# unirestore/UniRestore

Measured on AMD Instinct MI355X. Metric: restored 512x512 images/sec @ 20 denoise steps (whole job), higher is better.
Workload: dtype bf16; 1 GPU; PIR 512x512 batch=8/GPU, 20 DDIM steps, bf16, hipGraph replay (BASELINE.json configs[1]; configs[2] shape for N=8); global_batch=8, per_gpu_batch=8, image=512, denoise_steps=20, parallelism=image-parallel dp1, weights=seeded random init (no checkpoints reachable)

## Files before the change

### include/unirestore_hip.h

```cpp
#ifndef UNIRESTORE_HIP_H
#define UNIRESTORE_HIP_H

#include <stddef.h>
#include <stdint.h>

#ifdef __cplusplus
extern "C" {
#endif

typedef void* ur_stream_t;

enum { UR_OK = 0, UR_E_INVALID = -1, UR_E_UNSUPPORTED = -2, UR_E_LAUNCH = -3, UR_E_WORKSPACE = -4 };

enum { UR_DT_BF16 = 0, UR_DT_F16 = 1 };

enum {
  UR_ACT_NONE = 0,
  UR_ACT_SILU = 1,
  UR_ACT_GELU = 2,
  UR_ACT_GEGLU = 3,
  UR_ACT_GATE = 4,
  UR_ACT_TANH = 5,
  UR_ACT_RELU = 6
};
// ... 16 lines not shown
  const float* ln_stats;
  const float* ln_colsum;
  float ln_eps;
  int ln_dim;
  int ln_parts;
  float* workspace;
  size_t workspace_bytes;
  int N, H, W;
  int C1, ldx, C2, ldx2;
  int Cout, ldw, ldy, ldr;
  int KH, KW, stride, pad_t, pad_l;
  int OH, OW;
  int upsample2x;
  int act;
  int out_f32;
  int n_split, t_rows, t_ld;
  float out_scale;
  int nbatch;
  long long bs_x, bs_x2, bs_w, bs_bias, bs_y, bs_r;
  int k_chunk_major;
  long long bias_img_stride;
  int dtype;
  const void* w_frag;
} ur_conv_desc;

int ur_conv2d_nhwc(const ur_conv_desc* d, ur_stream_t stream);

typedef struct ur_conv_plan {
  int row_stat_parts;
  int gn_parts;
  int gn_fused;
  int prologue_ok;
} ur_conv_plan;
int ur_conv2d_plan(const ur_conv_desc* d, ur_conv_plan* plan);

typedef struct ur_conv_launch_info {
  int launcher;
  int splitk;
  int nk_per_split;
  int reduce;
  int reduce_ri;
  int gn_pass;
  int group_loop;
} ur_conv_launch_info;
int ur_conv2d_plan_launch(const ur_conv_desc* d, ur_conv_launch_info* info);
int ur_conv_launcher_count(void);
const char* ur_conv_launcher_name(int i);

int ur_gemm_bias_act(const void* x, const void* w, const float* bias, const void* residual, void* y, long long M, int N, int K,
                     int ldx, int ldw, int ldy, int ldr, int act, float* workspace, size_t workspace_bytes, int dtype,
                     ur_stream_t stream);
int ur_groupconv3x3_nhwc(const void* x, const void* w, const float* bias, void* y, int N, int H, int W, int Cg, int Cog,
                         int groups, int act, float* workspace, size_t workspace_bytes, int dtype, ur_stream_t stream);

int ur_groupnorm_stats_parts(int N, int HW, int C);
// ... 89 lines not shown
```

### unirestore_amd/build.py

```python
import json
import os
import re
import subprocess
import sys
from concurrent.futures import ThreadPoolExecutor

HERE = os.path.dirname(os.path.abspath(__file__))
CSRC = os.path.join(HERE, "csrc")
LIB = os.environ.get("UR_LIB_OUT") or os.path.join(HERE, "libunirestore_hip.so")
EXTRA = os.environ.get("UR_EXTRA_FLAGS", "").split()
IGEMM_UNITS = ["igemm_v2.hip", "igemm_halo.hip", "igemm_v1a.hip", "igemm_v1b.hip", "igemm_g1.hip"]
SOURCES = [(u, [f"-DUR_TU_F16={t}"], u.replace(".hip", "_f16.o" if t else "_bf16.o")) for u in IGEMM_UNITS for t in (0, 1)] + \
          [("conv_wstream.hip", [f"-DUR_TU_F16={t}"], "conv_wstream_f16.o" if t else "conv_wstream_bf16.o") for t in (0, 1)] + \
          [("attention.hip", [f"-DUR_TU_F16={t}"], "attention_f16.o" if t else "attention_bf16.o") for t in (0, 1)] + \
          [("attention_pp.hip", [f"-DUR_TU_F16={t}"], "attention_pp_f16.o" if t else "attention_pp_bf16.o") for t in (0, 1)] + \
          [("attention512.hip", [f"-DUR_TU_F16={t}"], "attention512_f16.o" if t else "attention512_bf16.o") for t in (0, 1)] + \
          [(u, [], u.replace(".hip", ".o")) for u in ("tchain.hip", "igemm.hip", "norms.hip", "elementwise.hip", "runtime.hip", "metrics.hip")]
FLAGS = ["--offload-arch=gfx950", "-O3", "-std=c++17", "-fPIC", "-Wno-unused-value",
         "-Wno-unused-result"]


def _hipcc():
    for c in ("/opt/rocm/bin/hipcc", "hipcc"):
        if os.path.isabs(c) and os.path.exists(c):
            return c
    return "hipcc"


def needs_build():
    if not os.path.exists(LIB):
        return True
    t = os.path.getmtime(LIB)
    deps = [os.path.join(CSRC, f) for f in os.listdir(CSRC)] + [os.path.join(HERE, "..", "include", "unirestore_hip.h")]
    return any(os.path.getmtime(d) > t for d in deps)
# ... 57 lines not shown
```

### unirestore_amd/capi.py

```python
import ctypes as C
import os

import torch

_HERE = os.path.dirname(os.path.abspath(__file__))
LIB_PATH = os.environ.get("UR_LIB") or os.path.join(_HERE, "libunirestore_hip.so")

UR_ACT_NONE, UR_ACT_SILU, UR_ACT_GELU, UR_ACT_GEGLU, UR_ACT_GATE, UR_ACT_TANH, UR_ACT_RELU = range(7)
UR_DT_BF16, UR_DT_F16 = 0, 1
UR_E_INVALID, UR_E_UNSUPPORTED = -1, -2


class ConvDesc(C.Structure):
    _fields_ = [
        ("x", C.c_void_p), ("x2", C.c_void_p), ("w", C.c_void_p), ("bias", C.c_void_p), ("residual", C.c_void_p),
        ("y", C.c_void_p), ("yt", C.c_void_p), ("gn_part", C.c_void_p), ("gn_ab", C.c_void_p), ("gn_silu", C.c_int),
        ("row_stats", C.c_void_p), ("ln_stats", C.c_void_p), ("ln_colsum", C.c_void_p), ("ln_eps", C.c_float), ("ln_dim", C.c_int), ("ln_parts", C.c_int),
        ("workspace", C.c_void_p),
        ("workspace_bytes", C.c_size_t),
        ("N", C.c_int), ("H", C.c_int), ("W", C.c_int),
        ("C1", C.c_int), ("ldx", C.c_int), ("C2", C.c_int), ("ldx2", C.c_int),
        ("Cout", C.c_int), ("ldw", C.c_int), ("ldy", C.c_int), ("ldr", C.c_int),
        ("KH", C.c_int), ("KW", C.c_int), ("stride", C.c_int), ("pad_t", C.c_int), ("pad_l", C.c_int),
        ("OH", C.c_int), ("OW", C.c_int),
        ("upsample2x", C.c_int), ("act", C.c_int), ("out_f32", C.c_int),
        ("n_split", C.c_int), ("t_rows", C.c_int), ("t_ld", C.c_int),
        ("out_scale", C.c_float),
        ("nbatch", C.c_int),
        ("bs_x", C.c_longlong), ("bs_x2", C.c_longlong), ("bs_w", C.c_longlong), ("bs_bias", C.c_longlong),
        ("bs_y", C.c_longlong), ("bs_r", C.c_longlong), ("k_chunk_major", C.c_int), ("bias_img_stride", C.c_longlong),
        ("dtype", C.c_int), ("w_frag", C.c_void_p),
    ]


class ConvPlan(C.Structure):
    _fields_ = [("row_stat_parts", C.c_int), ("gn_parts", C.c_int), ("gn_fused", C.c_int), ("prologue_ok", C.c_int)]


class ConvLaunchInfo(C.Structure):
    _fields_ = [("launcher", C.c_int), ("splitk", C.c_int), ("nk_per_split", C.c_int), ("reduce", C.c_int), ("reduce_ri", C.c_int),
                ("gn_pass", C.c_int), ("group_loop", C.c_int)]


_P, _I, _F, _LL, _SZ = C.c_void_p, C.c_int, C.c_float, C.c_longlong, C.c_size_t

SIGNATURES = {
    "ur_version": (_I, []),
    "ur_last_error": (C.c_char_p, []),
    "ur_conv2d_nhwc": (_I, [C.POINTER(ConvDesc), _P]),
    "ur_conv2d_plan": (_I, [C.POINTER(ConvDesc), C.POINTER(ConvPlan)]),
    "ur_conv2d_plan_launch": (_I, [C.POINTER(ConvDesc), C.POINTER(ConvLaunchInfo)]),
    "ur_conv_launcher_count": (_I, []),
    "ur_conv_launcher_name": (C.c_char_p, [_I]),
    "ur_gemm_bias_act": (_I, [_P, _P, _P, _P, _P, _LL, _I, _I, _I, _I, _I, _I, _I, _P, _SZ, _I, _P]),
    "ur_groupconv3x3_nhwc": (_I, [_P, _P, _P, _P, _I, _I, _I, _I, _I, _I, _I, _P, _SZ, _I, _P]),
    "ur_groupnorm_stats_parts": (_I, [_I, _I, _I]),
    "ur_groupnorm_ws_bytes": (_SZ, [_I, _I, _I]),
    "ur_groupnorm_ab_bytes": (_SZ, [_I, _I]),
    "ur_groupnorm_stats": (_I, [_P, _P, _I, _I, _I, _I, _P]),
# ... 82 lines not shown
```

### unirestore_amd/csrc/igemm.hip

```cpp
#include "igemm_impl.h"

namespace urk {
#define UR_DECLARE(name)                                                                                             \
  ConvLaunch name##_bf16(void* k, size_t ws_bytes);                                                                 \
  ConvLaunch name##_f16(void* k, size_t ws_bytes);                                                                  \
  static ConvLaunch name(ConvK& k, size_t ws_bytes) { return (k.f16 ? name##_f16 : name##_bf16)(&k, ws_bytes); }
UR_CONV_LAUNCHERS(UR_DECLARE)
#undef UR_DECLARE
}

namespace {

ConvLaunch dispatch_conv(ConvK& k, bool pair, size_t ws_bytes) {
  if (k.KH == 3 && k.stride == 1 && k.pad_t == 1 && k.pad_l == 1 && k.kcm && k.staged_ok_ && !pair && k.nbatch == 1 &&
      k.OW % 32 == 0 && k.OH % 8 == 0 && k.OH == (k.ups ? 2 * k.H : k.H) && k.OW == (k.ups ? 2 * k.W : k.W) && !k.yt) {
    const bool ok128 = k.Cout % 128 == 0, ok160 = k.Cout % 160 == 0;
    const long long tm8 = (long long)k.N * (k.OH / 8) * (k.OW / 32);
    auto eff = [](long long t) { return t <= 128 ? (double)(t * (256 / t)) / 256.0 : (double)t / (double)(((t + 255) / 256) * 256); };
    const bool use160 = ok160 && (!ok128 || eff(tm8 * (k.Cout / 160)) >= eff(tm8 * (k.Cout / 128)));
    const long long tiles8 = tm8 * (use160 ? k.Cout / 160 : k.Cout / 128);
    if ((ok128 || ok160) && tiles8 >= 64) {
      if (use160) return urk::halo_8x32_160(k, ws_bytes);
      return urk::halo_8x32_128(k, ws_bytes);
    }
  }
  if (k.KH == 3 && k.stride == 1 && k.pad_t == 1 && k.pad_l == 1 && k.kcm && !pair && k.nbatch == 1 && !k.ups && k.C2 == 0 &&
      k.Cout <= 32 && k.OW % 32 == 0 && k.OH % 8 == 0 && k.OH == k.H && k.OW == k.W && !k.yt && !k.gn_part && !k.gn_ab && !k.row_stats && !k.ln_stats &&
      !k.bias_img && (long long)k.N * (k.OH / 8) * (k.OW / 32) >= 128)
    return urk::halo_thin_32(k, ws_bytes);
  const bool himg_ups = k.ups && k.OH == 16 && k.OW == 16 && k.H == 8 && k.W == 8;
  if (k.KH == 3 && k.stride == 1 && k.pad_t == 1 && k.pad_l == 1 && k.kcm && k.staged_ok_ && !pair && k.nbatch == 1 &&
// ... 34 lines not shown
    if (k.Cout <= 32) return urk::v1_256x32(k, ws_bytes);
    if (k.Cout <= 64) return urk::v1_128x64(k, ws_bytes);
    if (k.Cout % 160 == 0 && k.Cout % 128 != 0) return g1 && nosplit(128, 160) ? urk::g1_128x160(k, ws_bytes) : urk::v1_128x160(k, ws_bytes);
    return g1 && nosplit(128, 128) ? urk::g1_128x128(k, ws_bytes) : urk::v1_128x128(k, ws_bytes);
  }
  if (k.Cout <= 32) return urk::v2_256x32(k, ws_bytes);
  if (k.Cout <= 64 && !pair) return urk::v2_128x64(k, ws_bytes);
  const bool n160 = !pair && k.Cout % 160 == 0 && k.Cout % 128 != 0;
  const long long big_tiles = (long long)((k.M + 255) / 256) * ((k.Cout + (n160 ? 159 : 127)) / (n160 ? 160 : 128)) * k.nbatch;
  if (g1 && !pair && big_tiles < 256) {
    const long long t160 = k.Cout % 160 == 0 ? (long long)((k.M + 127) / 128) * (k.Cout / 160) : 0;
    const long long t128 = (long long)((k.M + 127) / 128) * ((k.Cout + 127) / 128);
    auto fill = [](long long t) { return t <= 0 ? 0.0 : (double)t / (double)(((t + 255) / 256) * 256); };
    if (t160 >= 200 && fill(t160) >= fill(t128)) return urk::g1_128x160(k, ws_bytes);
    if (t128 >= 200) return urk::g1_128x128(k, ws_bytes);
  }
  if (big_tiles >= 160) {
    if (n160 && g1) return urk::g1_128x160(k, ws_bytes);
    if (n160) return urk::v2_256x160(k, ws_bytes);
    return urk::v2_256x128(k, ws_bytes);
  }
  if (k.Cout % 160 == 0 && k.Cout % 128 != 0 && !pair) return urk::v1_128x160(k, ws_bytes);
  return urk::v1_128x128(k, ws_bytes);
}

}

static int conv_impl(const ur_conv_desc* d, ur_stream_t stream, ur_conv_plan* plan, ur_conv_launch_info* info = nullptr) {
  UR_REQUIRE(d && d->x && d->w, "null x/w");
  UR_REQUIRE(d->KH == d->KW && (d->KH == 1 || d->KH == 3), "only 1x1 and 3x3 kernels");
  UR_REQUIRE(d->C1 > 0 && d->C1 % 8 == 0 && d->C2 % 8 == 0 && d->ldx % 8 == 0, "Cin/ldx must be multiples of 8");
  UR_REQUIRE(d->C2 == 0 || (d->x2 && d->ldx2 % 8 == 0), "virtual concat needs x2");
  UR_REQUIRE(d->Cout > 0 && d->Cout % 4 == 0 && d->ldw % 8 == 0, "Cout%4, ldw%8");
  UR_REQUIRE(d->nbatch >= 1 && d->stride >= 1 && d->OH > 0 && d->OW > 0, "bad dims");
  UR_REQUIRE(d->y || d->yt || d->gn_part, "no output requested");
  UR_REQUIRE_DT(d->dtype);
  const bool pair = d->act == UR_ACT_GEGLU || d->act == UR_ACT_GATE;
  if (pair && d->Cout % 64 != 0)
    return ur::fail(UR_E_UNSUPPORTED, "ur_conv2d_nhwc: pair activations (GEGLU / SimpleGate) need Cout % 64 == 0 (32-row a|g interleave)");
  UR_REQUIRE(!d->y || (d->out_f32 ? d->ldy % 4 == 0 : d->ldy % 4 == 0), "ldy%4");
  UR_REQUIRE(!d->residual || d->ldr % 4 == 0, "ldr%4");
  UR_REQUIRE(!d->yt || (d->t_rows > 0 && d->n_split % 4 == 0 && !pair), "bad transposed-output spec");

  ConvK k;
  k.x = (const uint16_t*)d->x; k.x2 = (const uint16_t*)d->x2; k.w = (const uint16_t*)d->w; k.bias = d->bias;
  k.res = (const uint16_t*)d->residual; k.y = d->y; k.yt = (uint16_t*)d->yt;
// ... 12 lines not shown

  k.kcm = d->k_chunk_major; k.wf = (const uint16_t*)d->w_frag; k.wmajor = 0; k.xgm = 0; k.xbn = 0; k.patch_tw = 0;
  UR_REQUIRE(!k.kcm || (k.Cin % 64 == 0 && d->C1 % 64 == 0), "k_chunk_major needs C1 and C1+C2 to be multiples of 64");
  k.gn_part = d->gn_part; k.gn_ab = d->gn_ab; k.gn_silu = d->gn_silu; k.f16 = d->dtype == UR_DT_F16; k.gn_fused = 0; k.gn_parts = 0;
  k.ln_parts = d->ln_parts;
  k.row_stats = d->row_stats; k.ln_stats = d->ln_stats; k.ln_colsum = d->ln_colsum; k.ln_eps = d->ln_eps; k.ln_dim = d->ln_dim;
  UR_REQUIRE(!d->ln_stats || (d->ln_colsum && d->ln_dim > 0), "ln_stats needs ln_colsum / ln_dim");
  UR_REQUIRE(!(d->bias_img_stride && (pair || d->ln_stats || d->yt)), "per-image bias rows do not combine with pair activations / LayerNorm folding / transposed columns");
  k.staged_ok_ = (d->y ? (!d->out_f32 && ((d->ldy | d->bs_y) & 7) == 0) : d->gn_part != nullptr) &&
                 (!d->residual || ((d->ldr | d->bs_r) & 7) == 0);
  UR_REQUIRE(!d->gn_part || (!d->out_f32 && !d->yt), "gn_part needs a plain 16-bit output (or none)");
  hipStream_t s = (hipStream_t)stream;
  const double flops = 2.0 * k.M * (double)k.Cout * k.Ktot * k.nbatch;
  const double bytes = 2.0 * ((double)k.M * k.Cin + (double)k.Cout * k.Ktot + (double)k.M * k.Cout) * k.nbatch;
  const char* fam = d->KH == 3 ? "conv3x3_igemm" : "gemm1x1_igemm";
  static const bool prof_shapes = getenv("UR_PROF_SHAPES") != nullptr;
  if (prof_shapes) {
    static std::map<std::string, int> interned;
    char buf[128];
    snprintf(buf, sizeof buf, "%s M%d N%d K%d s%d u%d b%d a%d", d->KH == 3 ? "c3" : "g1", k.M, k.Cout, k.Ktot, d->stride, d->upsample2x,
             k.nbatch, d->act);
    fam = interned.emplace(buf, 0).first->first.c_str();
  }
  const ConvLaunch launch = dispatch_conv(k, pair, d->workspace_bytes);
  const bool group_loop = k.nbatch > 1 && d->KH == 3 && k.kcm && k.stride == 1 && !pair && !k.gn_part && !k.row_stats && !k.ln_stats &&
                          !k.yt && !k.gn_ab && !k.out_f32 && k.staged_ok_ && k.Cout % 128 == 0 && !k.bias_img && k.C2 == 0;
  auto group_k = [&](int b) {
    ConvK kb = k;
    kb.nbatch = 1;
    kb.x = k.x + b * k.bs_x; kb.w = k.w + b * k.bs_w; kb.bias = k.bias ? k.bias + b * k.bs_bias : nullptr;
    kb.res = k.res ? k.res + b * k.bs_r : nullptr;
    kb.y = reinterpret_cast<uint16_t*>(k.y) + b * k.bs_y;
    kb.bs_x = kb.bs_w = kb.bs_bias = kb.bs_y = kb.bs_r = 0;
    return kb;
  };
  if (plan) {
    plan->row_stat_parts = d->row_stats ? (k.splitk > 1 ? 1 : k.tiles_n) : 0;
    plan->gn_parts = k.gn_parts; plan->gn_fused = k.gn_fused; plan->prologue_ok = launch.prologue_ok;
  }
  if (info) {
    ConvK kb = group_loop ? group_k(0) : k;
    const ConvLaunch l = group_loop ? dispatch_conv(kb, pair, d->workspace_bytes) : launch;
    info->launcher = l.id; info->splitk = kb.splitk; info->nk_per_split = kb.nk_per_split;
    const ReducePlan r = kb.splitk > 1 ? plan_splitk_reduce(kb) : ReducePlan{-1, 0};
    info->reduce = r.kind; info->reduce_ri = r.ri;
    info->gn_pass = k.gn_part && !k.gn_fused && !group_loop;
    info->group_loop = group_loop;
  }
  if (plan || info) return UR_OK;
  if (!d->y && d->gn_part && (!k.gn_fused || k.splitk > 1))
    return ur::fail(UR_E_UNSUPPORTED, "ur_conv2d_nhwc: y == NULL needs a launch whose epilogue writes gn_part (see ur_conv2d_plan)");
  if (d->gn_ab && !launch.prologue_ok)
    return ur::fail(UR_E_UNSUPPORTED, "ur_conv2d_nhwc: gn_ab is not supported by this launch (see ur_conv2d_plan.prologue_ok)");
  ur::ProfScope prof(fam, flops, bytes, s);
  UR_REQUIRE(!(d->row_stats || d->ln_stats) || (k.staged_ok_ && k.nbatch == 1 && !d->yt == !d->yt), "row_stats / ln fusion need a bf16 staged output");
  if (group_loop) {
    for (int b = 0; b < d->nbatch; ++b) {
      ConvK kb = group_k(b);
      const int rcb = dispatch_conv(kb, pair, d->workspace_bytes).launch(&kb, s);
      if (rcb != UR_OK) return rcb;
    }
    return UR_OK;
  }
  const int rc = launch.launch(&k, s);
  if (rc != UR_OK) return rc;
  if (k.gn_part && !k.gn_fused) {
    const int ctot = (pair ? k.Cout / 2 : k.Cout) * k.nbatch;
    UR_REQUIRE(k.y && k.ldy == ctot, "gn_part fallback needs a dense output (ldy == channels)");
    return ur::gn_stats_launch(k.y, k.gn_part, k.N, k.OHW, ctot, d->dtype, s);
  }
  return UR_OK;
}

extern "C" int ur_conv2d_nhwc(const ur_conv_desc* d, ur_stream_t stream) { return conv_impl(d, stream, nullptr); }

extern "C" int ur_conv2d_plan(const ur_conv_desc* d, ur_conv_plan* plan) {
// ... 45 lines not shown
```

### unirestore_amd/csrc/igemm_impl.h

```cpp
#pragma once
#include <cstdio>
#include <cstdlib>
#include <map>
#include <string>

#include "common.h"

static __device__ uint4 g_zero_page[8];
typedef uint32_t ig_u32x4 __attribute__((ext_vector_type(4)));

struct ConvLaunch {
  int (*launch)(void* k, hipStream_t s);
  int prologue_ok;
  int id;
};

namespace {

struct ConvK {
  const uint16_t* x; const uint16_t* x2; const uint16_t* w; const float* bias; const uint16_t* res;
  void* y; uint16_t* yt; float* ws; float* gn_part; const float* gn_ab;
  float* row_stats; const float* ln_stats; const float* ln_colsum; float ln_eps; int ln_dim, ln_parts;
  int N, H, W, C1, ldx, C2, ldx2, Cin, Cout, ldw, ldy, ldr, KH, KW, stride, pad_t, pad_l, OH, OW, OHW;
  int ups, act, out_f32, n_split, t_rows, t_ld;
  float out_scale;
  int M, Ktot, nk, tiles_m, tiles_n, splitk, nk_per_split, nbatch;
  long long bs_x, bs_x2, bs_w, bs_bias, bs_y, bs_r, bias_img;
  int gn_fused, gn_parts, gn_silu, f16, staged_ok_;
  int patch_tw;
  int kcm;
  const uint16_t* wf;
  int wmajor;
  int xgm, xbn;
};

__device__ __forceinline__ void xcd_tile_map(const ConvK& p, int id, int& tm, int& tn) {
  const int xcd = id & 7, idx = id >> 3;
  if (p.xgm) {
    const int lm = idx / p.xbn, ln = idx - lm * p.xbn;
    tm = (xcd % p.xgm) * (p.tiles_m / p.xgm) + lm;
    tn = (xcd / p.xgm) * p.xbn + ln;
    return;
  }
  const int nt = p.tiles_m * p.tiles_n, q = nt >> 3, r = nt & 7;
  id = (xcd < r ? xcd * (q + 1) : r * (q + 1) + (xcd - r) * q) + idx;
  if (p.wmajor) { tn = id / p.tiles_m; tm = id - tn * p.tiles_m; }
  else { tm = id / p.tiles_n; tn = id - tm * p.tiles_n; }
}

static inline void pick_xcd_grid(ConvK& k, double W, double A) {
  k.xgm = 0; k.xbn = 0; k.wmajor = 0;
  static const bool off = getenv("UR_NOXCDGRID") != nullptr;
  if (off || k.nbatch != 1) return;
  const long long nt = (long long)k.tiles_m * k.tiles_n;
  double best = 0.9 * (8.0 * W + A);
  if (nt % 8 == 0)
// ... 2180 lines not shown
```

### unirestore_amd/csrc/runtime.hip

```cpp
#include <cstring>
#include <mutex>
#include <sstream>
#include <vector>
#include <map>

#include "common.h"

namespace {
__global__ void zero_kernel(uint32_t* p, size_t n) {
  for (size_t i = blockIdx.x * (size_t)blockDim.x + threadIdx.x; i < n; i += (size_t)gridDim.x * blockDim.x) p[i] = 0u;
}
}

namespace ur {

void zero_async(void* ptr, size_t bytes, hipStream_t s) {
  const size_t n = bytes / 4;
  if (n == 0) return;
  const unsigned blocks = (unsigned)std::min<size_t>((n + 255) / 256, 1024);
  hipLaunchKernelGGL(zero_kernel, dim3(blocks), dim3(256), 0, s, (uint32_t*)ptr, n);
}

static thread_local std::string g_err;

// ... 29 lines not shown
  return e;
}

ProfScope::ProfScope(const char* family, double flops, double bytes, hipStream_t s) : slot(-1), stream(s) {
  if (!g_prof_on) return;
  hipStreamCaptureStatus st = hipStreamCaptureStatusNone;
  if (hipStreamIsCapturing(s, &st) != hipSuccess || st != hipStreamCaptureStatusNone) return;
  std::lock_guard<std::mutex> lk(g_mu);
  ProfRec r{family, flops, bytes, get_event(), get_event()};
  hipEventRecord(r.a, s);
  g_recs.push_back(r);
  slot = (int)g_recs.size() - 1;
}
ProfScope::~ProfScope() {
  if (slot < 0) return;
  std::lock_guard<std::mutex> lk(g_mu);
  hipEventRecord(g_recs[slot].b, stream);
}

}

extern "C" {

int ur_version(void) { return 101; }
const char* ur_last_error(void) { return ur::g_err.c_str(); }

int ur_profile_enable(int on) {
  std::lock_guard<std::mutex> lk(ur::g_mu);
  ur::g_prof_on = on != 0;
  if (on) {
    for (auto& r : ur::g_recs) {
      ur::g_pool.push_back(r.a);
      ur::g_pool.push_back(r.b);
    }
    ur::g_recs.clear();
  }
  return UR_OK;
}

int ur_profile_report(char* buf, size_t buf_bytes) {
  std::lock_guard<std::mutex> lk(ur::g_mu);
  struct Agg { long n = 0; double ms = 0, flops = 0, bytes = 0; };
  std::map<std::string, Agg> agg;
  for (auto& r : ur::g_recs) {
    hipEventSynchronize(r.b);
    float ms = 0.f;
    hipEventElapsedTime(&ms, r.a, r.b);
// ... 21 lines not shown
```

### unirestore_amd/modules/nn.py

```python
import math
from typing import Optional

import os

import torch
import torch.nn as nn

from .. import chain, ops
from ..ops import UR_ACT_GEGLU, UR_ACT_GELU, UR_ACT_NONE, UR_ACT_SILU

DEV = "cuda"
CHAIN = os.environ.get("UR_CHAIN", "1") == "1"


class _NoEager:
    def forward(self, *a, **k):
        raise RuntimeError(f"{type(self).__name__}: no eager/PyTorch path exists; use the HIP-backed graph")


class Conv2d(_NoEager, nn.Conv2d):
    def packed(self, pair=False, scale: Optional[torch.Tensor] = None) -> ops.PackedConv:
        key = ("pk", pair, ops.act_dtype())
        if key not in self.__dict__:
            w, b = self.weight, self.bias
            if scale is not None:
                s = scale.detach().reshape(-1)
                w = w * s[:, None, None, None]
                b = None if b is None else b * s
            self.__dict__[key] = ops.pack_conv(w, b, DEV, pair=pair, groups=self.groups)
        return self.__dict__[key]


class Linear(_NoEager, nn.Linear):
    def packed(self, pair=False) -> ops.PackedConv:
        key = ("pk", pair, ops.act_dtype())
# ... 233 lines not shown
        super().__init__()
        self.heads = heads
        kv_dim = kv_dim or c
        self.to_q = Linear(c, c, bias=False)
        self.to_k = Linear(kv_dim, c, bias=False)
        self.to_v = Linear(kv_dim, c, bias=False)
        self.to_out = _ToOut(c)

    def context_kv(self, ctx: torch.Tensor):
        key = ("cache", "ctx", ops.act_dtype())
        if key not in self.__dict__:
            tk = ctx.shape[1]
            c = self.to_q.out_features
            kv = _fused_qkv(self, ("to_k", "to_v"))
            vt = torch.zeros((1, c, ops.round_up(tk, 8)), dtype=ctx.dtype, device=DEV)
            k = ops.linear(ctx, kv, yt=vt, n_split=c, t_rows=tk)
            self.__dict__[key] = (k, vt, tk)
        return self.__dict__[key]

    def run_cross(self, h, ctx, residual, ln=None, rows=False):
        b, t, c = h.shape
        d = c // self.heads
        k, vt, tk = self.context_kv(ctx)
        if ln is not None:
            q = ops.linear(h, _fused_ln(self, "q", ("to_q",), ln[0]), ln_stats=ln[1])
        else:
            q = ops.linear(h, self.to_q.packed())
        o = ops.attention(q, k, vt, self.heads, d, t, tk, 1.0 / math.sqrt(d), ldq=c, ldk=2 * c, bs_q=t * c, bs_k=0,
                          bs_vt=0, batch=b)
        return ops.linear(o, self.to_out[0].packed(), residual=residual, rows=rows)


class GEGLU(nn.Module):
    def __init__(self, c, inner):
        super().__init__()
        self.proj = Linear(c, inner * 2)


class FeedForward(nn.Module):
    def __init__(self, c):
        super().__init__()
        self.net = nn.ModuleList([GEGLU(c, 4 * c), nn.Identity(), Linear(4 * c, c)])

    def run(self, h, residual, ln=None):
        if ln is not None:
            a = ops.linear(h, _fused_ln(self.net[0], "proj", ("proj",), ln[0], pair=True), ln_stats=ln[1], act=UR_ACT_GEGLU)
        else:
            a = ops.linear(h, self.net[0].proj.packed(pair=True), act=UR_ACT_GEGLU)
        return ops.linear(a, self.net[2].packed(), residual=residual)


class BasicTransformerBlock(nn.Module):
# ... 216 lines not shown
```

### unirestore_amd/ops.py

```python
from dataclasses import dataclass
from typing import Optional

import torch

from . import capi
from .capi import (UR_ACT_GATE, UR_ACT_GEGLU, UR_ACT_GELU, UR_ACT_NONE, UR_ACT_RELU, UR_ACT_SILU, UR_ACT_TANH, UR_DT_BF16,
                   UR_DT_F16, ConvDesc, ConvPlan, check, lib)

BF16 = torch.bfloat16
F16 = torch.float16
_ws = {}

_DTYPES = {"bf16": BF16, "bfloat16": BF16, BF16: BF16, "fp16": F16, "float16": F16, "f16": F16, "16": F16, F16: F16}
_act = BF16


def set_dtype(dt) -> torch.dtype:
    global _act
    if dt not in _DTYPES:
        raise ValueError(f"unsupported compute dtype {dt!r}: choose 'bf16' or 'fp16'")
    _act = _DTYPES[dt]
    return _act


# ... 123 lines not shown
    d.dtype = _dt(x)
    if plan_only:
        d.x, d.x2, d.w = 16, (16 if c2 else None), 16
    else:
        d.x, d.x2, d.w = _ptr(x), _ptr(x2), _ptr(pc.w)
    ws = workspace(x.device)
    d.workspace, d.workspace_bytes = ws.data_ptr(), ws.numel() * 4
    d.N, d.H, d.W = n, h, w_
    d.C1, d.ldx, d.C2, d.ldx2 = (c1 // g if g > 1 else c1), c1, c2, c2
    d.Cout, d.ldw, d.ldy = pc.cout // g, pc.w.shape[1], pc.cout_out
    d.KH = d.KW = k
    d.stride, d.pad_t, d.pad_l = stride, pad[0], pad[1]
    d.OH, d.OW = out_hw
    d.upsample2x, d.out_scale = int(upsample), 1.0
    d.k_chunk_major = int(pc.kcm and (c2 == 0 or c1 % 64 == 0))
    if wants_frag(pc, n, h, w_, c1, c2, stride, upsample, g) and pad == (1, 1):
        d.w_frag = 16 if plan_only else pc.frag().data_ptr()
    d.nbatch = g
    if g > 1:
        d.bs_x, d.bs_w, d.bs_bias, d.bs_y, d.bs_r = c1 // g, (pc.cout // g) * pc.w.shape[1], pc.cout // g, pc.cout_out // g, pc.cout_out // g
    return d


def conv(x: torch.Tensor, pc: PackedConv, *, x2=None, residual=None, bias=None, act=UR_ACT_NONE, stride=1, pad=None,
         out_hw=None, upsample=False, out_f32=False, out_scale=1.0, out=None, yt=None, n_split=0, t_rows=0,
         gn=False, store=True, rows=False, ln_stats=None, gn_ab=None, gn_silu=False):
    if x.dtype not in (BF16, F16) or x.dtype != pc.w.dtype or not x.is_contiguous() or x.dim() != 4:
        raise ValueError(f"conv: x must be a contiguous 4-d {pc.w.dtype} tensor, got {x.dtype} {tuple(x.shape)}")
    n, h, w_, c1 = x.shape
    c2 = 0 if x2 is None else x2.shape[-1]
    if (c1 + c2) != pc.cin * pc.groups:
        raise ValueError(f"conv: Cin mismatch: {c1}+{c2} vs {pc.cin}*{pc.groups}")
    d = _conv_desc(x, pc, x2, stride, pad, upsample, out_hw, plan_only=False)
    assert not pc.kcm or d.k_chunk_major, "chunk-major weights need a 64-aligned concat boundary"
    oh, ow = d.OH, d.OW
    co_total = pc.cout_out
    if out is None and store:
        out = torch.empty((n, oh, ow, co_total), dtype=torch.float32 if out_f32 else x.dtype, device=x.device)
    bias_t = pc.bias if bias is None else bias
    d.bias = _ptr(bias_t)
    if bias is not None and bias.dim() == 2 and bias.shape[0] > 1:
        d.bias_img_stride = bias.shape[1]
    d.residual, d.y, d.yt = _ptr(residual), _ptr(out), _ptr(yt)
    if ln_stats is not None:
        assert pc.ln_colsum is not None, "weights were not packed with pack_linear_ln"
        st, parts = ln_stats
        d.ln_stats, d.ln_colsum, d.ln_eps, d.ln_dim, d.ln_parts = st.data_ptr(), pc.ln_colsum.data_ptr(), pc.ln_eps, pc.cin, parts
    if gn_ab is not None:
        d.gn_ab, d.gn_silu = gn_ab.data_ptr(), int(gn_silu)
    if out is not None:
        d.ldy = out.shape[-1]
    d.ldr = residual.shape[-1] if residual is not None else 0
    d.act, d.out_f32, d.out_scale = act, int(out_f32), out_scale
    d.n_split, d.t_rows = n_split, t_rows
    d.t_ld = yt.shape[-1] if yt is not None else 0
    stats = rstats = None
    if gn or rows:
        if gn:
            d.gn_part = 16
        if rows:
            d.row_stats = 16
        plan = ConvPlan()
        check(lib.ur_conv2d_plan(d, plan))
        if gn:
            if not store and not plan.gn_fused:
                raise NotImplementedError("store=False needs a launch whose epilogue writes the statistics (conv_plan().gn_fused)")
            stats = (torch.empty((n, plan.gn_parts, co_total, 2), dtype=torch.float32, device=x.device), plan.gn_parts)
            d.gn_part = stats[0].data_ptr()
        if rows:
            rstats = (torch.empty((plan.row_stat_parts, n * oh * ow, 2), dtype=torch.float32, device=x.device), plan.row_stat_parts)
            d.row_stats = rstats[0].data_ptr()
    check(lib.ur_conv2d_nhwc(d, _stream()))
    if not store:
        return stats
    if stats is not None:
        out._gn = stats
    if rstats is not None:
        out._ln = rstats
# ... 415 lines not shown
```

Before: 30.67 images/s.

## Fuse cross-attention into the to_q GEMM epilogue

Adds a GEMM kernel variant whose epilogue runs the full cross-attention on the freshly computed Q tile. Each 64-column tile is one head, and K/V^T for up to 128 context tokens are staged in LDS, with softmax done online in registers. This removes the separate attention launch and the Q round-trip through global memory for the cross-attention blocks. The Python path uses it by default when the plan reports the fusion as eligible. In exchange it adds LDS pressure and an extra kernel template, and it only applies to narrow shape conditions.

```diff
diff --git a/include/unirestore_hip.h b/include/unirestore_hip.h
--- a/include/unirestore_hip.h
+++ b/include/unirestore_hip.h
@@ -62,6 +62,14 @@
   long long bias_img_stride;
   int dtype;
   const void* w_frag;
+  const void* xattn_k;
+  const void* xattn_vt;
+  long long xattn_bs_k, xattn_bs_vt;
+  int xattn_tk;
+  int xattn_ldk, xattn_ldvt;
+  int xattn_heads, xattn_head_dim;
+  int xattn_tq;
+  float xattn_scale;
 } ur_conv_desc;
 
 int ur_conv2d_nhwc(const ur_conv_desc* d, ur_stream_t stream);
@@ -71,6 +79,7 @@
   int gn_parts;
   int gn_fused;
   int prologue_ok;
+  int xattn_fused;
 } ur_conv_plan;
 int ur_conv2d_plan(const ur_conv_desc* d, ur_conv_plan* plan);
 
diff --git a/unirestore_amd/build.py b/unirestore_amd/build.py
--- a/unirestore_amd/build.py
+++ b/unirestore_amd/build.py
@@ -9,7 +9,7 @@
 CSRC = os.path.join(HERE, "csrc")
 LIB = os.environ.get("UR_LIB_OUT") or os.path.join(HERE, "libunirestore_hip.so")
 EXTRA = os.environ.get("UR_EXTRA_FLAGS", "").split()
-IGEMM_UNITS = ["igemm_v2.hip", "igemm_halo.hip", "igemm_v1a.hip", "igemm_v1b.hip", "igemm_g1.hip"]
+IGEMM_UNITS = ["igemm_v2.hip", "igemm_halo.hip", "igemm_v1a.hip", "igemm_v1b.hip", "igemm_g1.hip", "igemm_xattn.hip"]
 SOURCES = [(u, [f"-DUR_TU_F16={t}"], u.replace(".hip", "_f16.o" if t else "_bf16.o")) for u in IGEMM_UNITS for t in (0, 1)] + \
           [("conv_wstream.hip", [f"-DUR_TU_F16={t}"], "conv_wstream_f16.o" if t else "conv_wstream_bf16.o") for t in (0, 1)] + \
           [("attention.hip", [f"-DUR_TU_F16={t}"], "attention_f16.o" if t else "attention_bf16.o") for t in (0, 1)] + \
diff --git a/unirestore_amd/capi.py b/unirestore_amd/capi.py
--- a/unirestore_amd/capi.py
+++ b/unirestore_amd/capi.py
@@ -30,11 +30,15 @@
         ("bs_x", C.c_longlong), ("bs_x2", C.c_longlong), ("bs_w", C.c_longlong), ("bs_bias", C.c_longlong),
         ("bs_y", C.c_longlong), ("bs_r", C.c_longlong), ("k_chunk_major", C.c_int), ("bias_img_stride", C.c_longlong),
         ("dtype", C.c_int), ("w_frag", C.c_void_p),
+        ("xattn_k", C.c_void_p), ("xattn_vt", C.c_void_p), ("xattn_bs_k", C.c_longlong), ("xattn_bs_vt", C.c_longlong),
+        ("xattn_tk", C.c_int), ("xattn_ldk", C.c_int), ("xattn_ldvt", C.c_int), ("xattn_heads", C.c_int), ("xattn_head_dim", C.c_int),
+        ("xattn_tq", C.c_int), ("xattn_scale", C.c_float),
     ]
 
 
 class ConvPlan(C.Structure):
-    _fields_ = [("row_stat_parts", C.c_int), ("gn_parts", C.c_int), ("gn_fused", C.c_int), ("prologue_ok", C.c_int)]
+    _fields_ = [("row_stat_parts", C.c_int), ("gn_parts", C.c_int), ("gn_fused", C.c_int), ("prologue_ok", C.c_int),
+                ("xattn_fused", C.c_int)]
 
 
 class ConvLaunchInfo(C.Structure):
diff --git a/unirestore_amd/csrc/igemm.hip b/unirestore_amd/csrc/igemm.hip
--- a/unirestore_amd/csrc/igemm.hip
+++ b/unirestore_amd/csrc/igemm.hip
@@ -7,6 +7,8 @@
   static ConvLaunch name(ConvK& k, size_t ws_bytes) { return (k.f16 ? name##_f16 : name##_bf16)(&k, ws_bytes); }
 UR_CONV_LAUNCHERS(UR_DECLARE)
 #undef UR_DECLARE
+int (*xattn_launch_bf16(int id))(void*, hipStream_t);
+int (*xattn_launch_f16(int id))(void*, hipStream_t);
 }
 
 namespace {
@@ -87,6 +89,14 @@
   }
   if (k.Cout % 160 == 0 && k.Cout % 128 != 0 && !pair) return urk::v1_128x160(k, ws_bytes);
   return urk::v1_128x128(k, ws_bytes);
+}
+
+bool xattn_fuses(const ur_conv_desc* d, const ConvK& k, const ConvLaunch& launch, bool pair) {
+  const bool bn64 = launch.id == UR_LAUNCHER_g1_128x64 || launch.id == UR_LAUNCHER_g1_64x64 || launch.id == UR_LAUNCHER_g1_64x64_deep;
+  return d->xattn_k && d->xattn_vt && bn64 && k.splitk == 1 && k.nbatch == 1 && k.staged_ok_ && k.y && !pair && k.act == UR_ACT_NONE && !k.yt &&
+         !k.res && !k.gn_part && !k.row_stats && !k.bias_img && k.Cout % 64 == 0 && d->xattn_head_dim == 64 && d->xattn_heads * 64 == k.Cout &&
+         d->xattn_tk >= 1 && d->xattn_tk <= 128 && d->xattn_bs_k == 0 && d->xattn_bs_vt == 0 && d->xattn_ldk % 8 == 0 &&
+         d->xattn_ldvt % 8 == 0 && d->xattn_ldvt >= d->xattn_tk && d->xattn_tq > 0 && d->xattn_tq % 32 == 0 && k.M % d->xattn_tq == 0;
 }
 
 }
@@ -145,7 +155,15 @@
              k.nbatch, d->act);
     fam = interned.emplace(buf, 0).first->first.c_str();
   }
-  const ConvLaunch launch = dispatch_conv(k, pair, d->workspace_bytes);
+  k.xa_k = nullptr; k.xa_vt = nullptr; k.xa_tk = k.xa_ldk = k.xa_ldvt = 0; k.xa_scale_log2e = 0.f;
+  ConvLaunch launch = dispatch_conv(k, pair, d->workspace_bytes);
+  const bool xattn = xattn_fuses(d, k, launch, pair);
+  if (xattn) {
+    k.xa_k = (const uint16_t*)d->xattn_k; k.xa_vt = (const uint16_t*)d->xattn_vt;
+    k.xa_tk = d->xattn_tk; k.xa_ldk = d->xattn_ldk; k.xa_ldvt = d->xattn_ldvt;
+    k.xa_scale_log2e = (float)((double)d->xattn_scale * 1.4426950408889634);
+    launch.launch = (k.f16 ? urk::xattn_launch_f16 : urk::xattn_launch_bf16)(launch.id);
+  }
   const bool group_loop = k.nbatch > 1 && d->KH == 3 && k.kcm && k.stride == 1 && !pair && !k.gn_part && !k.row_stats && !k.ln_stats &&
                           !k.yt && !k.gn_ab && !k.out_f32 && k.staged_ok_ && k.Cout % 128 == 0 && !k.bias_img && k.C2 == 0;
   auto group_k = [&](int b) {
@@ -160,6 +178,7 @@
   if (plan) {
     plan->row_stat_parts = d->row_stats ? (k.splitk > 1 ? 1 : k.tiles_n) : 0;
     plan->gn_parts = k.gn_parts; plan->gn_fused = k.gn_fused; plan->prologue_ok = launch.prologue_ok;
+    plan->xattn_fused = xattn;
   }
   if (info) {
     ConvK kb = group_loop ? group_k(0) : k;
@@ -175,6 +194,8 @@
     return ur::fail(UR_E_UNSUPPORTED, "ur_conv2d_nhwc: y == NULL needs a launch whose epilogue writes gn_part (see ur_conv2d_plan)");
   if (d->gn_ab && !launch.prologue_ok)
     return ur::fail(UR_E_UNSUPPORTED, "ur_conv2d_nhwc: gn_ab is not supported by this launch (see ur_conv2d_plan.prologue_ok)");
+  if ((d->xattn_k || d->xattn_vt) && !xattn)
+    return ur::fail(UR_E_UNSUPPORTED, "ur_conv2d_nhwc: the xattn_* fields are not supported by this launch (see ur_conv2d_plan.xattn_fused)");
   ur::ProfScope prof(fam, flops, bytes, s);
   UR_REQUIRE(!(d->row_stats || d->ln_stats) || (k.staged_ok_ && k.nbatch == 1 && !d->yt == !d->yt), "row_stats / ln fusion need a bf16 staged output");
   if (group_loop) {
diff --git a/unirestore_amd/csrc/igemm_impl.h b/unirestore_amd/csrc/igemm_impl.h
--- a/unirestore_amd/csrc/igemm_impl.h
+++ b/unirestore_amd/csrc/igemm_impl.h
@@ -32,6 +32,9 @@
   const uint16_t* wf;
   int wmajor;
   int xgm, xbn;
+  const uint16_t* xa_k; const uint16_t* xa_vt;
+  int xa_tk, xa_ldk, xa_ldvt;
+  float xa_scale_log2e;
 };
 
 __device__ __forceinline__ void xcd_tile_map(const ConvK& p, int id, int& tm, int& tn) {
diff --git a/unirestore_amd/csrc/igemm_xattn.hip b/unirestore_amd/csrc/igemm_xattn.hip
--- /dev/null
+++ b/unirestore_amd/csrc/igemm_xattn.hip
@@ -0,0 +1,274 @@
+#include "igemm_impl.h"
+
+namespace {
+
+__device__ __forceinline__ int xa_swap23(int i) { return (i & 0x13) | ((i & 4) << 1) | ((i & 8) >> 1); }
+
+template <int BM> constexpr int xa_kv_offset() { return BM * (64 * 2 + 8) + 5 * 64 * 4 + BM * 8; }
+template <int BM, int NST> constexpr int xa_lds_bytes() {
+  constexpr int ring = NST * (BM + 64) * 128, epi = xa_kv_offset<BM>() + 2 * 16384;
+  return ring > epi ? ring : epi;
+}
+
+template <int BM, int NST, bool F16>
+__global__ __launch_bounds__(256) void gemm_xattn_kernel(const ConvK p) {
+  constexpr int BN = 64, WM = 2, WN = 2;
+  constexpr int NT = WM * WN * 64, RPP = NT / 8;
+  constexpr int WTM = BM / WM, WTN = BN / WN, FM = WTM / 32, FN = WTN / 32;
+  constexpr int XP = BM / RPP, WP = BN / RPP, NLD = XP + WP;
+  constexpr int STAGE = (BM + BN) * 128;
+  constexpr int SROW = BN * 2 + 8;
+  constexpr int KVOFF = xa_kv_offset<BM>();
+  static_assert(FN == 1 && (FM == 1 || FM == 2) && KVOFF % 128 == 0 && ktile_gemm_ok<FM, FN>(), "tile shape");
+  extern __shared__ __attribute__((aligned(16))) unsigned char smem[];
+  const int tid = threadIdx.x, lane = tid & 63, wid = tid >> 6;
+  const int wm = wid % WM, wn = wid / WM;
+  int tm, tn;
+  xcd_tile_map(p, blockIdx.x, tm, tn);
+  const int m0 = tm * BM, n0 = tn * BN;
+  const int lrow = tid >> 3;
+  const int chunk = (tid & 7) ^ ((lrow >> 1) & 7);
+  typedef __attribute__((address_space(1))) const void* gptr_t;
+  typedef __attribute__((address_space(3))) void* lptr_t;
+
+  int kbase = 0;
+  const ig_u32x4 rs_x = ig_make_rsrc(p.x, (unsigned long long)p.M * p.ldx * 2);
+  const ig_u32x4 rs_w = ig_make_rsrc(p.w, (unsigned long long)p.Cout * p.ldw * 2);
+  const unsigned smem_lds = (unsigned)(uintptr_t)(lptr_t)smem;
+  const int wid_s = __builtin_amdgcn_readfirstlane(wid);
+  unsigned xvo[XP], wvo[WP];
+#pragma unroll
+  for (int i = 0; i < XP; ++i) { const int m = m0 + i * RPP + lrow; xvo[i] = m < p.M ? ((unsigned)m * (unsigned)p.ldx + chunk * 8u) * 2u : IG_OOB; }
+#pragma unroll
+  for (int j = 0; j < WP; ++j) { const int r = n0 + j * RPP + lrow; wvo[j] = r < p.Cout ? ((unsigned)r * (unsigned)p.ldw + chunk * 8u) * 2u : IG_OOB; }
+  auto issue_tile = [&](int stage) {
+    const unsigned xs = smem_lds + stage * STAGE, wsm = xs + BM * 128;
+    const bool kval = kbase + chunk * 8 < p.Ktot;
+    const unsigned so = (unsigned)kbase * 2u;
+#pragma unroll
+    for (int i = 0; i < XP; ++i) ig_lds_dma16(xs + (i * RPP + wid_s * 8) * 128, kval ? xvo[i] : IG_OOB, rs_x, so);
+#pragma unroll
+    for (int j = 0; j < WP; ++j) ig_lds_dma16(wsm + (j * RPP + wid_s * 8) * 128, kval ? wvo[j] : IG_OOB, rs_w, so);
+    kbase += 64;
+  };
+  f32x16 acc[FN][FM];
+#pragma unroll
+  for (int b = 0; b < FM; ++b)
+#pragma unroll
+    for (int e = 0; e < 16; ++e) acc[0][b][e] = 0.f;
+  const int frow = lane & 31, fhalf = lane >> 5;
+  const unsigned kt_x0 = smem_lds + (wm * WTM + frow) * 128 + ((fhalf ^ ((frow >> 1) & 7)) << 4);
+  const unsigned kt_w0 = smem_lds + (BM + wn * WTN + frow) * 128 + ((fhalf ^ ((frow >> 1) & 7)) << 4);
+  const int ntile = p.nk;
+  int issued = 0;
+#pragma unroll
+  for (int s = 0; s < NST - 1; ++s)
+    if (issued < ntile) { issue_tile(s); ++issued; }
+  if (NST >= 3 && issued == NST - 1) asm volatile("s_waitcnt vmcnt(%0) lgkmcnt(0)" ::"n"(NLD * (NST >= 3 ? NST - 2 : 0)) : "memory");
+  else asm volatile("s_waitcnt vmcnt(0) lgkmcnt(0)" ::: "memory");
+  __builtin_amdgcn_s_barrier();
+  int cs = 0, is = (NST - 1) % NST;
+  for (int t = 0; t < ntile; ++t) {
+    if (issued < ntile) { issue_tile(is); ++issued; is = (is + 1 == NST) ? 0 : is + 1; }
+    unsigned ab[FM];
+#pragma unroll
+    for (int b = 0; b < FM; ++b) ab[b] = kt_x0 + cs * STAGE + b * 4096;
+    ktile_mma<FM, FN, F16>(acc, ab, kt_w0 + cs * STAGE);
+    cs = (cs + 1 == NST) ? 0 : cs + 1;
+    if (NST >= 3 && issued - (t + 1) >= NST - 1) asm volatile("s_waitcnt vmcnt(%0) lgkmcnt(0)" ::"n"(NLD * (NST >= 3 ? NST - 2 : 0)) : "memory");
+    else asm volatile("s_waitcnt vmcnt(0) lgkmcnt(0)" ::: "memory");
+    __builtin_amdgcn_s_barrier();
+  }
+  asm volatile("s_nop 15\n\ts_nop 7" ::: "memory");
+
+  const uint16_t* zero = reinterpret_cast<const uint16_t*>(g_zero_page);
+  const uint16_t* Kh = p.xa_k + n0;
+  const uint16_t* Vh = p.xa_vt + (long long)n0 * p.xa_ldvt;
+  const int ntk = (p.xa_tk + 63) >> 6;
+  {
+    const int lr = lane >> 3, ps = lane & 7;
+    for (int t = 0; t < ntk; ++t) {
+      unsigned char* ks = smem + KVOFF + t * 16384;
+      unsigned char* vs = ks + 8192;
+      const int kv0 = t * 64;
+#pragma unroll
+      for (int i = 0; i < 2; ++i) {
+        const int piece = wid + 4 * i, row = piece * 8 + lr;
+        const int ch = ps ^ ((row >> 1) & 7);
+        const uint16_t* g = kv0 + row < p.xa_tk ? Kh + (long long)(kv0 + row) * p.xa_ldk + ch * 8 : zero;
+        __builtin_amdgcn_global_load_lds((gptr_t)g, (lptr_t)(ks + piece * 1024), 16, 0, 0);
+      }
+#pragma unroll
+      for (int i = 0; i < 2; ++i) {
+        const int piece = wid + 4 * i, row = piece * 8 + lr;
+        const int ch = ps ^ ((row >> 1) & 7);
+        const uint16_t* g = kv0 + ch * 8 < p.xa_ldvt ? Vh + (long long)row * p.xa_ldvt + kv0 + ch * 8 : zero;
+        __builtin_amdgcn_global_load_lds((gptr_t)g, (lptr_t)(vs + piece * 1024), 16, 0, 0);
+      }
+    }
+  }
+
+  float* sbias = reinterpret_cast<float*>(smem + BM * SROW);
+  float* scol = sbias + 4 * BN;
+  float* srow = scol + BN;
+  const bool ln = p.ln_stats != nullptr;
+  for (int i = tid; i < BN; i += NT) sbias[i] = (p.bias && n0 + i < p.Cout) ? p.bias[n0 + i] : 0.f;
+  if (ln) {
+    for (int i = tid; i < BN; i += NT) scol[i] = n0 + i < p.Cout ? p.ln_colsum[n0 + i] : 0.f;
+    for (int r = tid; r < BM; r += NT) {
+      const int m = min(m0 + r, p.M - 1);
+      float sx = 0.f, sq = 0.f;
+      for (int q = 0; q < p.ln_parts; ++q) {
+        const float2 t2 = *reinterpret_cast<const float2*>(p.ln_stats + 2 * ((long long)q * p.M + m));
+        sx += t2.x; sq += t2.y;
+      }
+      const float mean = sx / p.ln_dim;
+      const float var = fmaxf(sq / p.ln_dim - mean * mean, 0.f);
+      srow[2 * r] = mean;
+      srow[2 * r + 1] = rsqrtf(var + p.ln_eps);
+    }
+  }
+  __syncthreads();
+  if (ln) epi_frag_pass<FM, FN, WTM, WTN, BM, BN, SROW, 0, 1, 0, 0, 0, F16>(p, acc, m0, n0, n0, wm, wn, lane, 0, smem, sbias, scol, srow);
+  else epi_frag_pass<FM, FN, WTM, WTN, BM, BN, SROW, 0, 0, 0, 0, 0, F16>(p, acc, m0, n0, n0, wm, wn, lane, 0, smem, sbias, scol, srow);
+  asm volatile("s_waitcnt vmcnt(0)" ::: "memory");
+  __syncthreads();
+
+  typedef typename Frag<F16>::type frag_t;
+  constexpr int DS = 4, NF = BM == 128 ? 2 : 1;
+  const int l31 = lane & 31, hf = lane >> 5;
+  const int g0 = BM == 128 ? wid * 32 : (wid >> 1) * 32;
+  const int f0 = BM == 128 ? 0 : (wid & 1);
+  frag_t qf[DS];
+  {
+    const unsigned char* qp = smem + (g0 + l31) * SROW + hf * 16;
+#pragma unroll
+    for (int ds = 0; ds < DS; ++ds) {
+      const uint2 a = *reinterpret_cast<const uint2*>(qp + ds * 32), b = *reinterpret_cast<const uint2*>(qp + ds * 32 + 8);
+      qf[ds] = __builtin_bit_cast(frag_t, make_uint4(a.x, a.y, b.x, b.y));
+    }
+  }
+  if (BM == 64) __syncthreads();
+  f32x16 oacc[NF];
+#pragma unroll
+  for (int f = 0; f < NF; ++f)
+#pragma unroll
+    for (int e = 0; e < 16; ++e) oacc[f][e] = 0.f;
+  float m_run = -1e30f, l_run = 0.f;
+  for (int t = 0; t < ntk; ++t) {
+    const unsigned char* ks = smem + KVOFF + t * 16384;
+    const unsigned char* vs = ks + 8192;
+    f32x16 sacc[2];
+#pragma unroll
+    for (int f = 0; f < 2; ++f) {
+#pragma unroll
+      for (int e = 0; e < 16; ++e) sacc[f][e] = 0.f;
+      const int row = f * 32 + xa_swap23(l31);
+      const int sw = (row >> 1) & 7;
+#pragma unroll
+      for (int ds = 0; ds < DS; ++ds) {
+        const frag_t kf = *reinterpret_cast<const frag_t*>(ks + row * 128 + (((ds * 2 + hf) ^ sw) << 4));
+        sacc[f] = mfma16t(kf, qf[ds], sacc[f]);
+      }
+    }
+    float s[32];
+#pragma unroll
+    for (int f = 0; f < 2; ++f)
+#pragma unroll
+      for (int r = 0; r < 16; ++r) s[f * 16 + r] = sacc[f][r];
+    if ((t + 1) * 64 > p.xa_tk) {
+#pragma unroll
+      for (int f = 0; f < 2; ++f)
+#pragma unroll
+        for (int r = 0; r < 16; ++r) {
+          const int key = t * 64 + f * 32 + 16 * (r >> 3) + 8 * hf + (r & 7);
+          if (key >= p.xa_tk) s[f * 16 + r] = -INFINITY;
+        }
+    }
+    float mx = s[0];
+#pragma unroll
+    for (int i = 1; i < 32; ++i) mx = fmaxf(mx, s[i]);
+    mx = fmaxf(mx, __shfl_xor(mx, 32, 64));
+    const float c = p.xa_scale_log2e;
+    if (!__all((mx - m_run) * c <= 8.0f)) {
+      const float m_new = fmaxf(m_run, mx);
+      const float alpha = __builtin_amdgcn_exp2f((m_run - m_new) * c);
+      l_run *= alpha;
+      m_run = m_new;
+#pragma unroll
+      for (int f = 0; f < NF; ++f)
+#pragma unroll
+        for (int e = 0; e < 16; ++e) oacc[f][e] *= alpha;
+    }
+    const float mc = m_run * c;
+    float psum = 0.f;
+#pragma unroll
+    for (int i = 0; i < 32; ++i) {
+      s[i] = __builtin_amdgcn_exp2f(fmaf(s[i], c, -mc));
+      psum += s[i];
+    }
+    l_run += psum;
+#pragma unroll
+    for (int kk = 0; kk < 4; ++kk) {
+      uint4 pk;
+      const float* sp = s + kk * 8;
+      pk.x = Act<F16>::pack2(sp[0], sp[1]); pk.y = Act<F16>::pack2(sp[2], sp[3]);
+      pk.z = Act<F16>::pack2(sp[4], sp[5]); pk.w = Act<F16>::pack2(sp[6], sp[7]);
+      const frag_t pf = __builtin_bit_cast(frag_t, pk);
+#pragma unroll
+      for (int f = 0; f < NF; ++f) {
+        const int row = (f0 + f) * 32 + l31;
+        const frag_t vf = *reinterpret_cast<const frag_t*>(vs + row * 128 + (((kk * 2 + hf) ^ ((row >> 1) & 7)) << 4));
+        oacc[f] = mfma16t(vf, pf, oacc[f]);
+      }
+    }
+  }
+  const float l_tot = l_run + __shfl_xor(l_run, 32, 64);
+  const float inv = 1.f / l_tot;
+  {
+    unsigned char* op = smem + (g0 + l31) * SROW;
+#pragma unroll
+    for (int f = 0; f < NF; ++f)
+#pragma unroll
+      for (int g = 0; g < 4; ++g) {
+        const int ch = (f0 + f) * 32 + 8 * g + 4 * hf;
+        *reinterpret_cast<uint2*>(op + ch * 2) =
+            make_uint2(Act<F16>::pack2(oacc[f][g * 4] * inv, oacc[f][g * 4 + 1] * inv),
+                       Act<F16>::pack2(oacc[f][g * 4 + 2] * inv, oacc[f][g * 4 + 3] * inv));
+      }
+  }
+  __syncthreads();
+  tile_copy<BM, BN, NT, SROW, false>(p, reinterpret_cast<uint16_t*>(p.y), p.ldy, smem, m0, p.M, n0, min(p.Cout, n0 + BN) - n0);
+}
+
+template <int BM, int NST>
+int xattn_launch(void* kp, hipStream_t s) {
+  ConvK& k = *static_cast<ConvK*>(kp);
+  constexpr int lds = xa_lds_bytes<BM, NST>();
+  static_assert(lds <= 160 * 1024, "LDS budget");
+  static ur::DeviceOnce attr_once;
+  if (auto once_guard = attr_once.first()) {
+    hipFuncSetAttribute(reinterpret_cast<const void*>(&gemm_xattn_kernel<BM, NST, UR_TU_F16 != 0>), hipFuncAttributeMaxDynamicSharedMemorySize, lds);
+  }
+  pick_xcd_grid(k, (double)k.Cout * k.Ktot, (double)k.M * k.Cin);
+  UR_F16_SWITCH(k, hipLaunchKernelGGL((gemm_xattn_kernel<BM, NST, F16>), dim3(k.tiles_m * k.tiles_n, 1, 1), dim3(256), lds, s, k));
+  return ur::check_launch("ur_conv2d_nhwc");
+}
+
+}
+
+#ifndef UR_NST_128x64
+#define UR_NST_128x64 2
+#endif
+#ifndef UR_NST_64x64
+#define UR_NST_64x64 2
+#endif
+
+namespace urk {
+int (*URK(xattn_launch)(int id))(void*, hipStream_t) {
+  if (id == UR_LAUNCHER_g1_128x64) return &xattn_launch<128, UR_NST_128x64>;
+  if (id == UR_LAUNCHER_g1_64x64) return &xattn_launch<64, UR_NST_64x64>;
+  if (id == UR_LAUNCHER_g1_64x64_deep) return &xattn_launch<64, 4>;
+  return nullptr;
+}
+}
diff --git a/unirestore_amd/csrc/runtime.hip b/unirestore_amd/csrc/runtime.hip
--- a/unirestore_amd/csrc/runtime.hip
+++ b/unirestore_amd/csrc/runtime.hip
@@ -75,7 +75,7 @@
 
 extern "C" {
 
-int ur_version(void) { return 101; }
+int ur_version(void) { return 102; }
 const char* ur_last_error(void) { return ur::g_err.c_str(); }
 
 int ur_profile_enable(int on) {
diff --git a/unirestore_amd/modules/nn.py b/unirestore_amd/modules/nn.py
--- a/unirestore_amd/modules/nn.py
+++ b/unirestore_amd/modules/nn.py
@@ -11,6 +11,7 @@
 
 DEV = "cuda"
 CHAIN = os.environ.get("UR_CHAIN", "1") == "1"
+XATTN_EPILOGUE = os.environ.get("UR_XATTN_EPILOGUE", "1") != "0"
 
 
 class _NoEager:
@@ -290,12 +291,15 @@
         b, t, c = h.shape
         d = c // self.heads
         k, vt, tk = self.context_kv(ctx)
-        if ln is not None:
-            q = ops.linear(h, _fused_ln(self, "q", ("to_q",), ln[0]), ln_stats=ln[1])
+        pq = _fused_ln(self, "q", ("to_q",), ln[0]) if ln is not None else self.to_q.packed()
+        lnkw = dict(ln_stats=ln[1]) if ln is not None else {}
+        xattn = (k, vt, tk, 1.0 / math.sqrt(d), self.heads, t)
+        if XATTN_EPILOGUE and ops.xattn_fuses(h, pq, xattn, ln=ln is not None):
+            o = ops.linear(h, pq, xattn=xattn, **lnkw)
         else:
-            q = ops.linear(h, self.to_q.packed())
-        o = ops.attention(q, k, vt, self.heads, d, t, tk, 1.0 / math.sqrt(d), ldq=c, ldk=2 * c, bs_q=t * c, bs_k=0,
-                          bs_vt=0, batch=b)
+            q = ops.linear(h, pq, **lnkw)
+            o = ops.attention(q, k, vt, self.heads, d, t, tk, 1.0 / math.sqrt(d), ldq=c, ldk=2 * c, bs_q=t * c, bs_k=0,
+                              bs_vt=0, batch=b)
         return ops.linear(o, self.to_out[0].packed(), residual=residual, rows=rows)
 
 
diff --git a/unirestore_amd/ops.py b/unirestore_amd/ops.py
--- a/unirestore_amd/ops.py
+++ b/unirestore_amd/ops.py
@@ -169,9 +169,31 @@
     return d
 
 
+def _set_xattn(d: ConvDesc, xattn, plan_only=False):
+    k, vt, tk, scale, heads, tq = xattn
+    d.xattn_k, d.xattn_vt = (16, 16) if plan_only else (k.data_ptr(), vt.data_ptr())
+    d.xattn_bs_k = k.stride(0) if k.dim() == 3 and k.shape[0] > 1 else 0
+    d.xattn_bs_vt = vt.stride(0) if vt.dim() == 3 and vt.shape[0] > 1 else 0
+    d.xattn_tk, d.xattn_ldk, d.xattn_ldvt = tk, k.shape[-1], vt.shape[-1]
+    d.xattn_heads, d.xattn_head_dim, d.xattn_tq, d.xattn_scale = heads, d.Cout // heads, tq, scale
+
+
+def xattn_fuses(x: torch.Tensor, pc: PackedConv, xattn, *, ln=False) -> bool:
+    rows = x.numel() // x.shape[-1]
+    d = _conv_desc(x.reshape(1, 1, rows, x.shape[-1]), pc, None, 1, None, False, None, plan_only=True)
+    d.y = 16
+    d.bias = 16 if pc.bias is not None else None
+    if ln:
+        d.ln_stats, d.ln_colsum, d.ln_eps, d.ln_dim, d.ln_parts = 16, 16, pc.ln_eps, pc.cin, 1
+    _set_xattn(d, xattn, plan_only=True)
+    plan = ConvPlan()
+    check(lib.ur_conv2d_plan(d, plan))
+    return bool(plan.xattn_fused)
+
+
 def conv(x: torch.Tensor, pc: PackedConv, *, x2=None, residual=None, bias=None, act=UR_ACT_NONE, stride=1, pad=None,
          out_hw=None, upsample=False, out_f32=False, out_scale=1.0, out=None, yt=None, n_split=0, t_rows=0,
-         gn=False, store=True, rows=False, ln_stats=None, gn_ab=None, gn_silu=False):
+         gn=False, store=True, rows=False, ln_stats=None, gn_ab=None, gn_silu=False, xattn=None):
     if x.dtype not in (BF16, F16) or x.dtype != pc.w.dtype or not x.is_contiguous() or x.dim() != 4:
         raise ValueError(f"conv: x must be a contiguous 4-d {pc.w.dtype} tensor, got {x.dtype} {tuple(x.shape)}")
     n, h, w_, c1 = x.shape
@@ -201,6 +223,8 @@
     d.act, d.out_f32, d.out_scale = act, int(out_f32), out_scale
     d.n_split, d.t_rows = n_split, t_rows
     d.t_ld = yt.shape[-1] if yt is not None else 0
+    if xattn is not None:
+        _set_xattn(d, xattn)
     stats = rstats = None
     if gn or rows:
         if gn:
```

New measurement: 30.85 images/s, median of 6. Within noise of the previous version (+0.6%).
